# gist-ailab/QuBER

Hardware: AMD Instinct MI355X
Metric: refined masks/sec on 640x480 RGB-D (N=20 inst) (higher is better)
Workload: dtype f32; 1 GPU; batch=16 640x480 RGB-D, 20 initial instances/frame, ResNet-50 RGB-D refiner (boundary-error -> fg/centre/offset), encode+network+grouping+mask extraction; parallelism=dp1, hipgraph=False, foreground_filter=False

## Files before the change

quber_amd/csrc/api_ops.hip:

```cpp
#include "plan.h"

using namespace quber;

static float* g_op_ws = nullptr;
static int g_op_skip_rows = 0;
static int g_op_bf16 = 0;
static const size_t g_op_ws_floats = (size_t)256 << 20;
static int g_op_wino_reuse = 0;

bool quber::op_set_tuning(int key, int value) {
    if (key == 2) {
        if (value && !g_op_ws) {
            if (hipMalloc((void**)&g_op_ws, sizeof(float) * g_op_ws_floats) != hipSuccess) g_op_ws = nullptr;
        } else if (!value && g_op_ws) {
            (void)hipFree(g_op_ws);
            g_op_ws = nullptr;
        }
        return true;
    }
    if (key == 26) { g_op_wino_reuse = value; return true; }
    if (key == 12) { g_op_bf16 = value; return true; }
    if (key == 11) { g_op_skip_rows = value; return true; }
    return false;
}
// ... 86 lines not shown
    p.bf16 = 2; p.es = 2;
    return launch_conv(p, 1, (hipStream_t)stream);
}

int quber_op_conv2d_f16(const void* x, int32_t B, int32_t h, int32_t w, int32_t cin, const void* w_packed, int32_t cout, int32_t ksize, int32_t stride, int32_t pad, int32_t dil,
                        int32_t kmode, const float* scale, const float* shift, const void* residual, int32_t relu, double* gn_sums, int32_t gn_groups, void* y, void* stream) {
    if (cin % 8 || (kmode && cin % 64)) return fail("conv2d_f16: cin must be a multiple of 8 (slice-major K order: of 64)");
    if (ksize < 1 || stride < 1 || dil < 1 || pad < 0) return fail("conv2d_f16: bad geometry");
    ConvP p{};
    p.in = (const float*)x; p.w = (const float*)w_packed; p.scale = scale; p.shift = shift; p.res = (const float*)residual; p.out = (float*)y;
    conv_geometry(p, B, h, w, cin, cout, ksize, stride, pad, dil);
    if (p.OH < 1 || p.OW < 1) return fail("conv2d_f16: empty output");
    p.res_cs = cout; p.Kpad = (p.K + 63) / 64 * 64; p.relu = relu;
    p.kmode = kmode; p.bf16 = 2; p.es = 2;
    p.w_gs = (long)cout * p.Kpad; p.ss_gs = cout;
    if (gn_sums) {
        if (gn_groups < 1 || cout % gn_groups) return fail("conv2d_f16: channels must divide into the norm groups");
        p.gn_sum = gn_sums; p.gn_groups = gn_groups; p.gn_cpg = cout / gn_groups;
    }
    return launch_conv(p, 1, (hipStream_t)stream);
}

int quber_op_conv1x1_dual(const float* y, const float* x, int32_t B, int32_t oh, int32_t ow, int32_t mid, int32_t h2, int32_t w2, int32_t cin, int32_t stride,
                          const float* w, const float* shift, const float* ones, int32_t cout, int32_t relu, float* out, void* stream) {
    ConvP p{};
    p.in = y; p.in2 = x; p.w = w; p.scale = ones; p.shift = shift; p.out = out;
    conv_geometry(p, B, oh, ow, mid, cout, 1, 1, 0, 1);
    p.H2 = h2; p.W2 = w2; p.in2_cs = cin; p.stride2 = stride; p.K1 = mid;
    p.K = mid + cin; p.Kpad = mid + cin; p.relu = relu;
    p.bf16 = g_op_bf16; p.ss_gs = 0;
    p.ws = g_op_ws; p.ws_floats = g_op_ws ? g_op_ws_floats : 0;
    if (g_op_bf16 == 3 && tune().x8) {
        static PlaneScratch scratch;
        const int rs = scratch.split(w, (long)cout * p.Kpad, p, "conv1x1_dual", (hipStream_t)stream);
        if (rs) return rs;
    }
    const int rc = launch_conv_dual(p, 1, (hipStream_t)stream);
    if (rc == 1) return fail("conv1x1_dual: launch not covered by the dual kernel (workspace: tuning key 2)");
    return rc;
}

int quber_op_conv3x3_winograd(const float* x, int32_t B, int32_t h, int32_t w, int32_t cin, const float* w_oihw, int32_t cout, int32_t dil, int32_t m,
                              const float* scale, const float* shift, int32_t relu, float* u, float* ws, int64_t ws_floats, float* y, void* stream) {
    hipStream_t st = (hipStream_t)stream;
    if (!winograd_eligible(3, 1, dil, dil, cin, cout)) return fail("winograd: unsupported channel counts");
    if ((scale == nullptr) != (shift == nullptr)) return fail("winograd: scale and shift go together");
    if (m != 2 && m != 4 && m != 6) return fail("winograd: the output tile edge is 2, 4 or 6");
    int rc = g_op_wino_reuse ? 0 : launch_winograd_weights(w_oihw, cout, cin, m, u, st);
    if (rc) return rc;
    WinoP q{};
    q.in = mkview(x, B, h, w, cin); q.out = mkview(y, B, h, w, cout);
    q.u = u; q.scale = scale; q.shift = shift; q.ss_gs = 0; q.relu = relu; q.dil = dil; q.m = m;
    q.dtype = g_op_bf16;
    q.ws = ws; q.ws_floats = (size_t)ws_floats;
    if (m == 4 && tune().wino_fused && cout % 32 == 0 && (size_t)ws_floats >= (size_t)36 * cout * cin) {
        q.uf = ws;
        if (winograd_fused_ok(q, B, 1)) {
            rc = winograd_fused_prepare();
            if (rc) return rc;
            rc = g_op_wino_reuse ? 0 : launch_winograd_fused_pack(u, cout, cin, ws, st);
            if (rc) return rc;
            q.ws = ws + (size_t)36 * cout * cin; q.ws_floats = (size_t)ws_floats - (size_t)36 * cout * cin;
        } else {
            q.uf = nullptr;
        }
    }
    q.splitk_ws = g_op_ws; q.splitk_floats = g_op_ws ? g_op_ws_floats : 0;
    return launch_conv_winograd(q, B, 1, st);
}

int quber_op_groupnorm(const float* x, int32_t B, int32_t h, int32_t w, int32_t c, int32_t groups, const float* gamma,
                       const float* beta, float eps, int32_t relu, double* stats, float* y, void* stream) {
    View in = mkview(x, B, h, w, c), out = mkview(y, B, h, w, c);
    int rc = launch_gn_stats(in, B, 1, groups, stats, (hipStream_t)stream);
    if (rc) return rc;
    return launch_gn_apply(in, out, B, 1, groups, stats, gamma, beta, 0, eps, relu, (hipStream_t)stream);
}

int quber_op_bilinear(const float* x, int32_t B, int32_t h, int32_t w, int32_t c, int32_t oh, int32_t ow, float* y,
                      void* stream) {
    if (c % 4) return fail("bilinear: channels must be a multiple of 4");
    return launch_bilinear(mkview(x, B, h, w, c), mkview(y, B, oh, ow, c), B, (hipStream_t)stream);
}

int quber_op_group_pixels(const float* logits, int32_t n_planes, int32_t batch, int32_t h, int32_t w, int32_t cap,
                          const int32_t* centers, const int32_t* ncenters, uint8_t* ids, uint32_t* area, void* stream) {
    if (!logits || !centers || !ncenters || !ids || !area || batch < 1 || h < 1 || w < 1) return fail("bad argument to quber_op_group_pixels");
    return launch_group_pixels(logits, n_planes, batch, h, w, cap, centers, ncenters, ids, area, (hipStream_t)stream);
}

int quber_op_maxpool3x3s2(const float* x, int32_t B, int32_t h, int32_t w, int32_t c, float* y, void* stream) {
    if (c % 4) return fail("maxpool: channels must be a multiple of 4");
    return launch_maxpool3x3s2(mkview(x, B, h, w, c), mkview(y, B, (h + 1) / 2, (w + 1) / 2, c), B, 1, (hipStream_t)stream);
}

}
```

quber_amd/csrc/common.h:

```cpp
#pragma once
#include <hip/hip_runtime.h>
#include <stdint.h>
#include <string>

namespace quber {

struct View {
    float* p = nullptr;
    int B = 0, H = 0, W = 0, C = 0;
    int cs = 0;
    long gs = 0;
    int es = 4;
    float* at(long elems) const { return p ? reinterpret_cast<float*>(reinterpret_cast<char*>(p) + elems * es) : nullptr; }
};

struct ConvP {
    const float* in;
    const float* w;
    const float* scale;
    const float* shift;
    const float* res;
    const float* prelu;
    float* out;
    int B, H, W, Cin, in_cs;
// ... 21 lines not shown
    const char* tag;
    int pk_T, pk_tpg, pk_min, pk_in_bytes, pk_debug;
    const float* in2;
    int in2_cs, H2, W2, stride2, K1, pk_in2_bytes;
    long in2_gs;
    int es;
    int acc_chunk;
    int lean_in_bytes;
    unsigned dv_m[5], dv_s[5];
    const void* w3;
    long w3_plane;
    int dil_g[4];
    int h8_ss_bytes;
    const double* n_stats; const float* n_gamma; const float* n_beta; float* n_coef;
    int n_groups, n_param_gs, n_relu, n_coef_bytes; float n_eps;
    int bf16;
    int zones, zx1, zx2;
};

int device_cus();
void set_error(const std::string& msg);
int fail(const std::string& msg);

struct ProfScope {
    int rec;
    hipStream_t st;
    ProfScope(const char* tag, double bytes, double flops, hipStream_t s);
    ~ProfScope();
    ProfScope(const ProfScope&) = delete;
    ProfScope& operator=(const ProfScope&) = delete;
};

struct WinoNorm {
    const double* stats;
    const float* gamma;
    const float* beta;
    int groups, cpg, param_gs, relu;
    double n;
    float eps;
};

struct WinoP {
    View in, out;
    const float* u;
    const void* u3;
    long u3_plane;
    const float* uf;
    int algo;
    const float* scale;
    const float* shift;
    int ss_gs, relu;
    int dil;
    int m;
    int dtype;
    double* gn_sum;
    int gn_groups;
    WinoNorm norm;
    float* ws;
    size_t ws_floats;
    float* splitk_ws;
    size_t splitk_floats;
};

int launch_conv(const ConvP& p, int G, hipStream_t st);
int launch_conv_winograd(const WinoP& q, int B, int G, hipStream_t st);
int launch_winograd_weights(const float* w_oihw, int Cout, int Cin, int m, float* u, hipStream_t st);
void winograd_weights_host(const float* w_oihw, int Cout, int Cin, int m, float* u);
bool winograd_eligible(int k, int stride, int pad, int dil, int Cin, int Cout);
bool winograd_m6_channels_ok(int Cin, int Cout);
size_t winograd_ws_floats(int B, int H, int W, int Cin, int Cout, int G, int dil, int m);
double winograd_mac_ratio(int H, int W, int dil, int m);
bool winograd_fused_ok(const WinoP& q, int B, int G);
int launch_conv_winograd_fused(const WinoP& q, int B, int G, hipStream_t st);
void winograd_fused_pack_host(const float* u, int Cout, int Cin, float* uf);
int launch_winograd_fused_pack(const float* u, int Cout, int Cin, float* uf, hipStream_t st);
size_t winograd_fused_ws_floats(int B, int Cin, int G);
int winograd_fused_prepare();

struct Tuning {
    int winograd = 0;
    int wino_min_cin = 32;
    int wino_max_ratio = 67;
    int wino_variant = 0;
    int wino_min_cout = 32;
    int wino_pairs = 0;
    int wino_chunk_mb = 0;
    int wino_fused = 1;
    int wino_fused_max_cin = 160;
    int acc_chunk = 2;
    int tile_128x64 = 1;
    int force_tile = 0;
    int force_split = 0;
    int tail_split = 1;
    int persist = 1;
    int persist_min_nk = 32;
    int persist_min_tiles = 256;
    int persist_debug = 0;
    int stem_fused = 1;
    int lean_loader = 1;
    int fuse_shortcut = 1;
    int lanes = 1;
    int h8 = 1;
    int x8 = 1;
    int x8_min_nk = 8;
    int x8_min_rounds = 2;
    int zone_cols = 1;
    int small_n_64 = 1;
    int aspp_lanes = 1;
    int h8_narrow = 1;
    int h8_norm = 1;
    int h8_min_tiles = 224;
};
extern Tuning g_tune;
extern thread_local const Tuning* t_tune;
inline const Tuning& tune() { return t_tune ? *t_tune : g_tune; }
struct TuneScope {
    const Tuning* prev;
    explicit TuneScope(const Tuning* t) : prev(t_tune) { t_tune = t; }
    ~TuneScope() { t_tune = prev; }
    TuneScope(const TuneScope&) = delete;
    TuneScope& operator=(const TuneScope&) = delete;
};
bool tuning_set(Tuning& t, int key, int value);
template <int BM, int BN, int WM, int WN> int launch_conv_persistent(ConvP p, int G, int bpc, hipStream_t st);
size_t conv_persistent_ws_floats(int BM, int BN, int bpc);
bool conv_persistent_ok(const ConvP& p);
int conv_persistent_segments(int T, int P, int nk, int min_slices, int bid, int* out4, int cap);
int conv_persistent_fixup(int T, int P, int nk, int min_slices, int xcd, int j, int* tile, int* slots, int cap);
int launch_conv_dual(ConvP p, int G, hipStream_t st);
bool conv_h8_patch_takes(const ConvP& p, int G, bool norm);
int launch_conv_x8(ConvP p, int G, hipStream_t st);
int launch_split_bf16x3(const float* w, long n, void* planes, hipStream_t st);
int launch_conv_h8(ConvP p, int G, hipStream_t st);
#ifdef PK_STAMPS
int pk_read_stamps(unsigned long long* dst, int n);
int pk_read_span(unsigned long long* dst, int n);
#endif
int launch_preprocess(const uint8_t* rgb, const uint8_t* depth, const float* offs, const View& x, int B, int Bcap,
                      int H, int W, const float* mean6, const float* std6, int streams, hipStream_t st);
// ... 110 lines not shown
```

quber_amd/csrc/plan.hip:

```cpp
#include "plan.h"

namespace quber {
namespace {

constexpr int BLOCKS50[4] = {3, 4, 6, 3}, BLOCKS101[4] = {3, 4, 23, 3}, BLOCKS152[4] = {3, 8, 36, 3};

struct BnFold {
    const float *w, *b, *m, *v;
    bool ok() const { return w && b && m && v; }
    float scale(int o) const { return w[o] * (1.0f / sqrtf(v[o] + 1e-5f)); }
    float shift(int o, float sc) const { return b[o] - m[o] * sc; }
};
BnFold frozen_bn(Builder& b, const std::string& n, int C) {
    return {b.hw(n + ".norm.weight", C), b.hw(n + ".norm.bias", C), b.hw(n + ".norm.running_mean", C), b.hw(n + ".norm.running_var", C)};
}

struct WinoChoice { bool take = false; int m = 0; double ratio = 0.0; bool one_kernel = false; };
WinoChoice choose_winograd(int H, int W, int k, int stride, int pad, int dil, int Cin, int Cout, bool plain, int dtype) {
    WinoChoice r;
    if (!winograd_eligible(k, stride, pad, dil, Cin, Cout) || !plain || tune().winograd == 1 || (dtype != 0 && dtype != 3)) return r;
    const double lim = (double)tune().wino_max_ratio / 100.0;
    const double r6 = winograd_m6_channels_ok(Cin, Cout) ? winograd_mac_ratio(H, W, dil, 6) : 1e9;
    const double r4 = winograd_mac_ratio(H, W, dil, 4), r2 = winograd_mac_ratio(H, W, dil, 2);
    double best = lim;
// ... 83 lines not shown
    const int K = k * k * Cin, Kpad = (K + KS - 1) / KS * KS;
    const int OH = (in.H + 2 * pad - dil * (k - 1) - 1) / stride + 1;
    const int OW = (in.W + 2 * pad - dil * (k - 1) - 1) / stride + 1;
    const bool skip_rows = k == 3 && stride == 1 && dil > 1 && Cin % KS == 0 && cin_real == Cin && 10 * 2 * pad >= 2 * 3 * OH &&
                           !(winograd_eligible(k, stride, pad, dil, Cin, out.C) && !res && prelu.empty() &&
                             std::min(winograd_mac_ratio(in.H, in.W, dil, 4), winograd_mac_ratio(in.H, in.W, dil, 2)) <= tune().wino_max_ratio / 100.0 && tune().winograd != 1);
    const int kmode = (k > 1 && Cin % KS == 0 && !skip_rows) ? 1 : 0;
    if (dry) return;
    const double fl = 2.0 * OH * OW * (double)cin_real * k * k * Cout * G;
    c->flops += fl;
    if (OH != out.H || OW != out.W) { if (err.empty()) err = "internal: conv output geometry mismatch at " + name; return; }
    for (const float* p : w)
        if (!p) return;
    std::vector<float> packed((size_t)G * Cout * Kpad, 0.f);
    for (int g = 0; g < G; ++g)
        for (int o = 0; o < Cout; ++o) {
            float* dst = &packed[((size_t)g * Cout + o) * Kpad];
            for (int ci = 0; ci < cin_real; ++ci)
                for (int t = 0; t < k * k; ++t) {
                    const size_t kk = kmode ? ((size_t)(ci / KS) * k * k + t) * KS + ci % KS : (size_t)t * Cin + ci;
                    dst[kk] = w[g][((size_t)o * cin_real + ci) * k * k + t];
                }
        }
    ConvP p{};
    p.in = in.p;
    p.w = upload_weights(packed);
    if (aes != 2 && k == 1) { p.w3 = split3(p.w, packed.size()); p.w3_plane = (long)packed.size(); }
    p.es = aes;
    if (in.es != aes || out.es != aes || (res && res->es != aes)) { if (err.empty()) err = "internal: element type mismatch at " + name; return; }
    const bool ident = !affine && aes == 2 && Cout >= 32;
    p.scale = affine ? upload(scale) : ident ? upload(std::vector<float>((size_t)G * Cout, 1.f)) : nullptr;
    p.shift = affine ? upload(shift) : ident ? upload(std::vector<float>((size_t)G * Cout, 0.f)) : nullptr;
    for (size_t g = 0; g < dil_g.size() && g < 4; ++g) p.dil_g[g] = dil_g[g];
    p.prelu = prelu.empty() ? nullptr : upload(prelu);
    p.res = res ? res->p : nullptr;
    p.out = out.p;
    p.H = in.H; p.W = in.W; p.Cin = Cin; p.in_cs = in.cs;
    p.OH = OH; p.OW = OW; p.Cout = Cout; p.out_cs = out.cs;
    p.res_cs = res ? res->cs : 0;
    p.K = K; p.Kpad = Kpad;
    p.kh = k; p.kw = k; p.stride = stride; p.pad = pad; p.dil = dil;
    p.relu = relu; p.kmode = kmode; p.skip_rows = skip_rows;
    p.bf16 = c->cfg.compute_dtype;
    p.in_gs = in.gs; p.out_gs = out.gs; p.res_gs = res ? res->gs : 0;
    p.w_gs = (long)Cout * Kpad; p.ss_gs = Cout;
    p.ohw = OH * OW;
    quber_ctx* ctx = c;
    const WinoChoice wc = choose_winograd(in.H, in.W, k, stride, pad, dil, Cin, Cout, cin_real == Cin && !res && prelu.empty(), c->cfg.compute_dtype);
    const bool wino = wc.take;
    WinoP wq{};
    if (wino) {
        const int m = wc.m, P = (m + 2) * (m + 2);
        c->wino_flops += fl;
        c->wino_saved += fl * (1.0 - wc.ratio);
        c->wino_pad += fl * (wc.ratio - (double)((m + 2) * (m + 2)) / (9.0 * m * m));
        std::vector<float> u((size_t)G * P * Cout * Cin);
        for (int g = 0; g < G; ++g) winograd_weights_host(w[g], Cout, Cin, m, &u[(size_t)g * P * Cout * Cin]);
        wq.in = in; wq.out = out; wq.u = upload(u);
        wq.u3 = split3(wq.u, u.size()); wq.u3_plane = (long)u.size();
        if (wc.one_kernel) {
            std::vector<float> uf(u.size());
            for (int g = 0; g < G; ++g) winograd_fused_pack_host(&u[(size_t)g * P * Cout * Cin], Cout, Cin, &uf[(size_t)g * P * Cout * Cin]);
            wq.uf = upload(uf);
        }
        wq.scale = p.scale; wq.shift = p.shift; wq.ss_gs = Cout; wq.relu = relu; wq.dil = dil; wq.m = m;
        wq.dtype = c->cfg.compute_dtype;
    }
    std::shared_ptr<DeferredNorm> norm, norm16;
    if (wino && pending_norm && pending_norm->out.p == in.p && pending_norm->C == Cin && pending_norm->G == G) {
        norm = pending_norm;
        norm->absorbed = true;
    }
    float* coef16 = nullptr;
    if (!wino && aes == 2 && tune().h8_norm && tune().h8 && tune().h8_narrow && pending_norm && pending_norm->out.p == in.p && pending_norm->C == Cin &&
        pending_norm->G == G && k == 3 && stride == 1 && pad == 1 && dil == 1 && dil_g.empty() && Cin % 64 == 0 && Cin >= 128 && Cin <= 512 && cin_real == Cin &&
        (Cout == 128 || Cout == 64 || Cout == 32 || (Cout >= 256 && Cout % 8 == 0 && tune().h8_narrow != 2)) && !res && prelu.empty() && in.cs == pending_norm->in.cs && in.gs == pending_norm->in.gs) {
        norm16 = pending_norm;
        norm16->absorbed = true;
        coef16 = (float*)dalloc_bytes(sizeof(float) * (size_t)G * Bmax * Cin * 2);
    }
    pending_norm.reset();
    if (wino) {
        WinoP probe = wq;
        if (norm) probe.in = norm->in;
        const bool fusedk = wq.uf && winograd_fused_ok(probe, Bmax, G);
        wq.algo = fusedk ? 2 : 1;
        if (wq.uf && winograd_fused_prepare() && err.empty()) err = "winograd (fused): cannot raise the kernels' LDS limit";
        const size_t need = fusedk ? winograd_fused_ws_floats(Bmax, Cin, G) : winograd_ws_floats(Bmax, in.H, in.W, Cin, Cout, G, dil, wq.m);
        if (need > c->wino_floats) c->wino_floats = need;
        if (cur_lane) {
            const int lb = std::min(Bmax, LANE_BATCH);
            const size_t ln = fusedk ? winograd_fused_ws_floats(lb, Cin, G) : winograd_ws_floats(lb, in.H, in.W, Cin, Cout, G, dil, wq.m);
            if (ln > c->lane_wino_floats[cur_lane]) c->lane_wino_floats[cur_lane] = ln;
        }
    }
    auto fuse = std::make_shared<GnFuse>();
    last_conv = {fuse, out.p, G, Cout};
    const int L = cur_lane;
    c->ops.push_back({[p, G, ctx, fuse, wq, wino, norm, norm16, coef16, L](int B, hipStream_t st) mutable {
        const bool side = L && ctx->lane_now == L;
        float* const sk_ws = side ? ctx->lane_splitk_ws[L] : ctx->splitk_ws;
        const size_t sk_floats = side ? ctx->lane_splitk_floats : ctx->splitk_floats;
        if (wino) {
            wq.ws = side ? ctx->lane_wino_ws[L] : ctx->wino_ws; wq.ws_floats = side ? ctx->lane_wino_floats[L] : ctx->wino_floats;
            wq.splitk_ws = sk_ws; wq.splitk_floats = sk_floats;
            wq.gn_sum = fuse->sums; wq.gn_groups = fuse->groups;
            if (norm) {
                wq.in = norm->in;
                wq.norm = WinoNorm{norm->stats, norm->gamma, norm->beta, 32, 0, norm->C, 1, 0.0, 1e-5f};
            }
            return launch_conv_winograd(wq, B, G, st);
        }
        p.B = B;
        p.M = B * p.OH * p.OW;
        p.ws = sk_ws;
        p.ws_floats = sk_floats;
        p.gn_sum = fuse->sums;
        p.gn_groups = fuse->groups;
        p.gn_cpg = fuse->groups ? p.Cout / fuse->groups : 0;
        if (norm16) {
            ConvP q = p;
            q.in = norm16->in.p;
            q.n_stats = norm16->stats; q.n_gamma = norm16->gamma; q.n_beta = norm16->beta; q.n_coef = coef16;
            q.n_groups = 32; q.n_param_gs = norm16->C; q.n_relu = 1; q.n_eps = 1e-5f;
            if (conv_h8_patch_takes(q, G, true)) return launch_conv(q, G, st);
            const int rc = launch_gn_apply(norm16->in, norm16->out, B, G, 32, norm16->stats, norm16->gamma, norm16->beta, norm16->C, 1e-5f, 1, st);
            if (rc) return rc;
        }
        return launch_conv(p, G, st);
    }, OP_CONV, name, fl, 1});
    c->ops.back().lane = cur_lane;
}

void Builder::conv(const std::vector<std::string>& names, const View& in, int cin_real, const View& out, int k, int stride, int pad, int dil, Affine af, const View* res, bool relu,
                   const std::vector<int>& dil_g) {
    const int G = (int)names.size(), Cout = out.C;
    std::vector<float> scale((size_t)G * Cout, 1.f), shift((size_t)G * Cout, 0.f);
    std::vector<const float*> w;
    for (int g = 0; g < G; ++g) {
// ... 469 lines not shown
```

quber_amd/csrc/runtime.hip:

```cpp
#include <atomic>

#include "plan.h"

namespace quber {

Tuning g_tune;
thread_local const Tuning* t_tune = nullptr;

struct TuneKey { int key; int Tuning::*field; bool plan; };
constexpr TuneKey TUNE_KEYS[] = {
    {3, &Tuning::force_split, false},           {4, &Tuning::force_tile, false},
    {5, &Tuning::tail_split, false},            {6, &Tuning::winograd, true},
    {7, &Tuning::wino_min_cin, true},           {8, &Tuning::wino_max_ratio, true},
    {9, &Tuning::wino_variant, true},           {10, &Tuning::wino_min_cout, true},
    {13, &Tuning::persist, false},              {14, &Tuning::persist_min_nk, false},
    {15, &Tuning::persist_min_tiles, false},    {16, &Tuning::persist_debug, false},
    {17, &Tuning::wino_pairs, false},           {18, &Tuning::fuse_shortcut, true},
    {19, &Tuning::tile_128x64, false},          {20, &Tuning::wino_chunk_mb, false},
    {21, &Tuning::acc_chunk, false},            {24, &Tuning::lanes, false},
    {25, &Tuning::wino_fused, true},            {27, &Tuning::wino_fused_max_cin, true},
    {29, &Tuning::stem_fused, true},            {30, &Tuning::lean_loader, false},
    {31, &Tuning::h8, false},                   {32, &Tuning::h8_min_tiles, false},
    {35, &Tuning::x8, false},                   {36, &Tuning::x8_min_rounds, false},
    {37, &Tuning::x8_min_nk, false},            {38, &Tuning::h8_narrow, false},
    {39, &Tuning::h8_norm, true},               {41, &Tuning::aspp_lanes, true},
    {42, &Tuning::small_n_64, false},           {43, &Tuning::zone_cols, false},
};
int* tuning_field(Tuning& t, int key) {
    for (const TuneKey& k : TUNE_KEYS)
        if (k.key == key) return &(t.*k.field);
    return nullptr;
}
bool tuning_set(Tuning& t, int key, int value) {
    int* f = tuning_field(t, key);
    if (f) *f = value;
    return f != nullptr;
}
bool tuning_plan_time(int key) {
    for (const TuneKey& k : TUNE_KEYS)
        if (k.key == key) return k.plan;
    return false;
}

int device_cus() {
    static std::atomic<int> cache[64];
    int dev = 0;
    if (hipGetDevice(&dev) != hipSuccess) return -1;
    const bool cached = dev >= 0 && dev < 64;
    if (cached) {
        const int v = cache[dev].load(std::memory_order_relaxed);
        if (v > 0) return v;
    }
    hipDeviceProp_t prop;
    if (hipGetDeviceProperties(&prop, dev) != hipSuccess) return -1;
    const int cus = prop.multiProcessorCount > 0 ? prop.multiProcessorCount : 256;
    if (cached) cache[dev].store(cus, std::memory_order_relaxed);
    return cus;
}

static thread_local std::string g_err;
extern "C" const char* quber_last_error(void) { return g_err.c_str(); }
void set_error(const std::string& m) { g_err = m; }
int fail(const std::string& m) { g_err = m; return -1; }

thread_local Profiler* g_prof = nullptr;

ProfScope::ProfScope(const char* tag, double bytes, double flops, hipStream_t s) : rec(-1), st(s) {
    Profiler* p = g_prof;
    if (!p) return;
    int ti = -1;
    for (size_t i = 0; i < p->tags.size(); ++i)
        if (p->tags[i] == tag) { ti = (int)i; break; }
    if (ti < 0) { ti = (int)p->tags.size(); p->tags.emplace_back(tag); }
    ProfRec r{ti, p->get(), p->get(), bytes, flops};
    if (!r.e0 || !r.e1 || hipEventRecord(r.e0, s) != hipSuccess) return;
    rec = (int)p->recs.size();
    p->recs.push_back(r);
}
ProfScope::~ProfScope() {
// ... 5 lines not shown
```

quber_amd/csrc/winograd.hip:

```cpp
#include "common.h"
#include "winograd_xf.h"

namespace quber {

using namespace wxf;


namespace {

#ifndef QB_WINO_IN_WAVES44
#define QB_WINO_IN_WAVES44 2
#endif
constexpr int wino_in_waves(int O, int V) { return O == 4 ? (V == 4 ? QB_WINO_IN_WAVES44 : 5) : O == 2 ? 4 : 2; }
constexpr int wino_out_waves(int O, int V) { return O == 4 ? (V == 4 ? 2 : 3) : O == 2 ? 4 : 1; }

template <int O, int V, bool NORM>
__global__ __launch_bounds__(256) __attribute__((amdgpu_waves_per_eu(wino_in_waves(O, V)))) void wino_input_kernel(const float* __restrict__ in, int B, int H, int W, int CV, int in_cs,
                                                         long in_gs, int TH, int TW, int d, float* __restrict__ v, long v_gs,
                                                         const WinoNorm np, int Ball, int boff) {
    constexpr int T = O + 2;
    using VT = Vec<V>;
    const int g = blockIdx.z;
    in += g * in_gs;
    v += g * v_gs;
    const int tpb = 256 / CV;
    const int cv = tpb ? threadIdx.x % CV : blockIdx.y * 256 + threadIdx.x;
    const long tiles = (long)B * d * d * TH * TW;
    const int nblk = gridDim.x, xcd = blockIdx.x & 7, bq = nblk >> 3, br = nblk & 7;
    const int vb = (xcd < br ? xcd * (bq + 1) : br * (bq + 1) + (xcd - br) * bq) + (blockIdx.x >> 3);
    const long tile = tpb ? (long)vb * tpb + threadIdx.x / CV : vb;
    if (tile >= tiles || cv >= CV || (tpb && (int)(threadIdx.x / CV) >= tpb)) return;
    const TileAt ta = locate(tile, TH, TW, d);
    const int c = cv * V;
    const float* base = in + (long)ta.b * H * W * in_cs + c;
    VT nsc, nbi;
    if constexpr (NORM) {
        const double* sb = np.stats + (((long)g * Ball + boff + ta.b) * np.groups + c / np.cpg) * 2;
        const double mean = sb[0] / np.n;
        double var = sb[1] / np.n - mean * mean;
        if (var < 0.0) var = 0.0;
        const float rstd = (float)(1.0 / sqrt(var + (double)np.eps));
        const VT ga = vload<V>(np.gamma + g * np.param_gs + c), be = vload<V>(np.beta + g * np.param_gs + c);
#pragma unroll
        for (int e = 0; e < V; ++e) {
            nsc.v[e] = rstd * ga.v[e];
            nbi.v[e] = be.v[e] - (float)mean * nsc.v[e];
        }
    }
    const float relu_lo = (NORM && np.relu) ? 0.f : -__builtin_inff();
    VT t[T][T];
#pragma unroll
    for (int j = 0; j < T; ++j) {
        const int x = d * (O * ta.tx - 1 + j) + ta.px;
        VT col[T], tc[T];
        const int xc = min(max(x, 0), W - 1);
        const bool xin = (unsigned)x < (unsigned)W;
#pragma unroll
        for (int i = 0; i < T; ++i) {
            const int y = d * (O * ta.ty - 1 + i) + ta.py;
            col[i] = vload<V>(base + ((long)min(max(y, 0), H - 1) * W + xc) * in_cs);
        }
#pragma unroll
        for (int i = 0; i < T; ++i) {
            const int y = d * (O * ta.ty - 1 + i) + ta.py;
            const bool inside = xin && (unsigned)y < (unsigned)H;
#pragma unroll
            for (int e = 0; e < V; ++e) {
                float q = col[i].v[e];
                if constexpr (NORM) q = fmaxf(fmaf(q, nsc.v[e], nbi.v[e]), relu_lo);
                col[i].v[e] = inside ? q : 0.f;
            }
        }
        bt<O>(col, tc);
#pragma unroll
        for (int i = 0; i < T; ++i) t[i][j] = tc[i];
    }
    float* dst = v + tile * (long)(CV * V) + c;
    const long ps = tiles * (long)(CV * V);
#pragma unroll
    for (int i = 0; i < T; ++i) {
        VT row[T];
        bt<O>(t[i], row);
#pragma unroll
        for (int j = 0; j < T; ++j) vstore<V>(dst + (i * T + j) * ps, row[j]);
    }
}

constexpr int OUT_ITERS = 4;
template <int O, int V>
__global__ __launch_bounds__(256) __attribute__((amdgpu_waves_per_eu(wino_out_waves(O, V)))) void wino_output_kernel(const float* __restrict__ m, long m_gs, int B, int OH, int OW, int CV,
                                                          int TH, int TW, int d, const float* __restrict__ scale,
                                                          const float* __restrict__ shift, int ss_gs, int relu,
                                                          float* __restrict__ out, int out_cs, long out_gs,
                                                          double* __restrict__ gn_sum, int gn_groups, int gn_cpg, int Ball, int boff, int iters) {
    constexpr int T = O + 2;
    using VT = Vec<V>;
    const int g = blockIdx.z;
    m += g * m_gs;
    out += g * out_gs;
    const int tpb = 256 / CV;
    const int cv = tpb ? threadIdx.x % CV : blockIdx.y * 256 + threadIdx.x;
    const int c = cv * V;
    const long per_img = (long)d * d * TH * TW;
    const long tiles = (long)B * per_img;
    const int step = tpb ? tpb : 1;
    const long tile0 = (long)blockIdx.x * step * iters;
    const bool lane_ok = cv < CV && (!tpb || (int)(threadIdx.x / CV) < tpb);
    __shared__ double gacc[2 * 32 * 2];
    const int b0 = (int)(tile0 / per_img);
    if (gn_sum) {
        if (threadIdx.x < 128) gacc[threadIdx.x] = 0.0;
        __syncthreads();
    }
    double s0 = 0.0, q0 = 0.0, s1 = 0.0, q1 = 0.0;
    const long ps = tiles * (long)(CV * V);
    VT sc, sh;
    if (scale && lane_ok) {
        sc = vload<V>(scale + g * ss_gs + c);
        sh = vload<V>(shift + g * ss_gs + c);
    }
    for (int it = 0; it < iters; ++it) {
        const long tile = tile0 + (long)it * step + (tpb ? threadIdx.x / CV : 0);
        if (!lane_ok || tile >= tiles) continue;
        const TileAt ta = locate(tile, TH, TW, d);
        const float* src = m + tile * (long)(CV * V) + c;
        VT s[O][T];
#pragma unroll
        for (int j = 0; j < T; ++j) {
            VT col[T], sj[O];
#pragma unroll
            for (int i = 0; i < T; ++i) col[i] = vload<V>(src + (i * T + j) * ps);
            at<O>(col, sj);
#pragma unroll
            for (int i = 0; i < O; ++i) s[i][j] = sj[i];
        }
        double a = 0.0, q = 0.0;
#pragma unroll
        for (int i = 0; i < O; ++i) {
            const int oy = d * (O * ta.ty + i) + ta.py;
            VT row[O];
            at<O>(s[i], row);
            if (oy >= OH) continue;
#pragma unroll
            for (int j = 0; j < O; ++j) {
                const int ox = d * (O * ta.tx + j) + ta.px;
                if (ox >= OW) continue;
                VT y = row[j];
#pragma unroll
                for (int e = 0; e < V; ++e) {
                    if (scale) y.v[e] = fmaf(y.v[e], sc.v[e], sh.v[e]);
                    if (relu) y.v[e] = fmaxf(y.v[e], 0.f);
                    a += (double)y.v[e];
                    q += (double)y.v[e] * y.v[e];
                }
                vstore<V>(out + (((long)ta.b * OH + oy) * OW + ox) * out_cs + c, y);
            }
        }
        if (ta.b == b0) { s0 += a; q0 += q; } else { s1 += a; q1 += q; }
    }
    if (gn_sum) {
        if (lane_ok) {
            const int grp = c / gn_cpg;
            if (s0 != 0.0 || q0 != 0.0) { atomicAdd(&gacc[grp * 2], s0); atomicAdd(&gacc[grp * 2 + 1], q0); }
            if (s1 != 0.0 || q1 != 0.0) { atomicAdd(&gacc[64 + grp * 2], s1); atomicAdd(&gacc[64 + grp * 2 + 1], q1); }
        }
        __syncthreads();
        if (threadIdx.x < 128) {
            const double v = gacc[threadIdx.x];
            const int b = b0 + (threadIdx.x >> 6);
            if (v != 0.0 && b < B) atomicAdd(&gn_sum[(((long)g * Ball + boff + b) * gn_groups) * 2 + (threadIdx.x & 63)], v);
        }
    }
}

template <int O>
__host__ __device__ inline void gmul(double a, double b, double c, double* y) {
    if constexpr (O == 2) {
        y[0] = a;
        y[1] = 0.5 * (a + b + c);
        y[2] = 0.5 * (a - b + c);
        y[3] = c;
    } else if constexpr (O == 4) {
        y[0] = a * (64.0 / 81.0);
        y[1] = -a * (128.0 / 243.0) - b * (32.0 / 81.0) - c * (8.0 / 27.0);
        y[2] = -a * (128.0 / 243.0) + b * (32.0 / 81.0) - c * (8.0 / 27.0);
        y[3] = a * (32.0 / 243.0) + b * (16.0 / 81.0) + c * (8.0 / 27.0);
        y[4] = a * (32.0 / 243.0) - b * (16.0 / 81.0) + c * (8.0 / 27.0);
        y[5] = c;
    } else {
        y[0] = a;
        y[1] = -(a + b + c) * (2.0 / 9.0);
        y[2] = -(a - b + c) * (2.0 / 9.0);
        y[3] = a / 90.0 + b / 45.0 + c * (2.0 / 45.0);
        y[4] = a / 90.0 - b / 45.0 + c * (2.0 / 45.0);
        y[5] = (32.0 * a + 16.0 * b + 8.0 * c) / 45.0;
        y[6] = (32.0 * a - 16.0 * b + 8.0 * c) / 45.0;
        y[7] = c;
    }
}
// ... 15 lines not shown
    constexpr int P = (O + 2) * (O + 2);
    const long n = (long)Cout * Cin;
    for (long i = blockIdx.x * (long)blockDim.x + threadIdx.x; i < n; i += (long)gridDim.x * blockDim.x) {
        double up[P];
        wino_filter<O>(w + i * 9, up);
        for (int p = 0; p < P; ++p) u[p * n + i] = (float)up[p];
    }
}

template <int O>
void weights_host(const float* w_oihw, int Cout, int Cin, float* u) {
    constexpr int P = (O + 2) * (O + 2);
    for (int o = 0; o < Cout; ++o)
        for (int c = 0; c < Cin; ++c) {
            double up[P];
            wino_filter<O>(w_oihw + ((size_t)o * Cin + c) * 9, up);
            for (int p = 0; p < P; ++p) u[((size_t)p * Cout + o) * Cin + c] = (float)up[p];
        }
}

}

void winograd_weights_host(const float* w_oihw, int Cout, int Cin, int m, float* u) {
    if (m == 6) weights_host<6>(w_oihw, Cout, Cin, u);
    else if (m == 4) weights_host<4>(w_oihw, Cout, Cin, u);
    else weights_host<2>(w_oihw, Cout, Cin, u);
}

int launch_winograd_weights(const float* w_oihw, int Cout, int Cin, int m, float* u, hipStream_t st) {
    if (m == 6) hipLaunchKernelGGL(wino_weight_kernel<6>, dim3(256), dim3(256), 0, st, w_oihw, Cout, Cin, u);
    else if (m == 4) hipLaunchKernelGGL(wino_weight_kernel<4>, dim3(256), dim3(256), 0, st, w_oihw, Cout, Cin, u);
    else hipLaunchKernelGGL(wino_weight_kernel<2>, dim3(256), dim3(256), 0, st, w_oihw, Cout, Cin, u);
    QB_CHECK(hipGetLastError());
    return 0;
}

bool winograd_m6_channels_ok(int Cin, int Cout) {
    return (Cin / 2 <= 256 || (Cin / 2) % 256 == 0) && (Cout / 2 <= 256 || (Cout / 2) % 256 == 0);
}

bool winograd_eligible(int k, int stride, int pad, int dil, int Cin, int Cout) {
    return k == 3 && stride == 1 && dil >= 1 && pad == dil && Cin % 32 == 0 && Cout % 4 == 0 && Cin >= tune().wino_min_cin &&
           Cout >= tune().wino_min_cout && (Cin / 4 <= 256 || (Cin / 4) % 256 == 0) && (Cout / 4 <= 256 || (Cout / 4) % 256 == 0);
}

size_t winograd_ws_floats(int B, int H, int W, int Cin, int Cout, int G, int dil, int m) {
    const size_t tiles = (size_t)B * wino_tiles(H, W, dil, m);
    return (size_t)G * (m + 2) * (m + 2) * tiles * (size_t)(Cin + Cout);
}

double winograd_mac_ratio(int H, int W, int dil, int m) {
    return (double)((m + 2) * (m + 2)) * wino_tiles(H, W, dil, m) / (9.0 * H * W);
}


template <int O, int V>
static int run_winograd(const WinoP& q, int Ball, int G, hipStream_t st) {
    constexpr int P = (O + 2) * (O + 2);
    const View& in = q.in;
    const View& out = q.out;
    const int H = in.H, W = in.W, Cin = in.C, Cout = out.C, d = q.dil;
    const int TH = tiles_1d(H, d, O), TW = tiles_1d(W, d, O);
    const long tiles_pf = wino_tiles(H, W, d, O);
    if ((long)Ball * tiles_pf * P >= (1L << 31) / 2) return fail("winograd: too many tiles");
    int cb = Ball;
    if (tune().wino_chunk_mb > 0) {
        const double per_frame = 4.0 * G * P * (double)tiles_pf * (Cin + Cout);
        cb = (int)((double)tune().wino_chunk_mb * 1048576.0 / per_frame);
        if (cb < 1) cb = 1;
        if (cb > Ball) cb = Ball;
        cb = (Ball + (Ball + cb - 1) / cb - 1) / ((Ball + cb - 1) / cb);
    }
    if (winograd_ws_floats(cb, H, W, Cin, Cout, G, d, O) > q.ws_floats) return fail("winograd: workspace too small");
    WinoNorm np = q.norm;
    if (np.stats) {
        if (np.groups <= 0 || Cin % np.groups || (Cin / np.groups) % 4) return fail("winograd: fused GroupNorm needs 4 | channels per group");
        np.cpg = Cin / np.groups;
        np.n = (double)H * W * np.cpg;
    }
    const int CVo = Cout / V, per_iter = CVo <= 256 ? 256 / CVo : 1;
    int iters = OUT_ITERS;
    {
        const long groups = CVo <= 256 ? ((long)Ball * tiles_pf + per_iter - 1) / per_iter : (long)Ball * tiles_pf * (CVo / 256);
        while (iters > 1 && groups * G / iters < 2048) iters >>= 1;
    }
    const bool gn_here = q.gn_sum && q.gn_groups > 0 && q.gn_groups <= 32 && (Cout / q.gn_groups) % 4 == 0 &&
                         tiles_pf >= (long)per_iter * iters;
    for (int b0 = 0; b0 < Ball; b0 += cb) {
        const int B = Ball - b0 < cb ? Ball - b0 : cb;
        const long tiles = (long)B * tiles_pf;
        float* v = q.ws;
        auto grid = [&](int CV) {
            return CV <= 256 ? dim3((unsigned)((tiles + 256 / CV - 1) / (256 / CV)), 1, G) : dim3((unsigned)tiles, CV / 256, G);
        };
        const float* in_p = in.p + (size_t)b0 * H * W * in.cs;
        float* out_p = out.p + (size_t)b0 * H * W * out.cs;
        const bool shared_v = G > 1 && in.gs == 0 && !np.stats;
        const int Gv = shared_v ? 1 : G;
        float* m = q.ws + (size_t)Gv * P * tiles * Cin;
        auto grid_v = [&](int CV) {
            return CV <= 256 ? dim3((unsigned)((tiles + 256 / CV - 1) / (256 / CV)), 1, Gv) : dim3((unsigned)tiles, CV / 256, Gv);
        };
        {
            ProfScope prof("wino_input", 4.0 * Gv * Cin * ((double)B * H * W + (double)P * tiles), 0.0, st);
            if (np.stats)
                hipLaunchKernelGGL((wino_input_kernel<O, V, true>), grid_v(Cin / V), dim3(256), 0, st, in_p, B, H, W, Cin / V, in.cs, in.gs, TH,
                                   TW, d, v, (long)P * tiles * Cin, np, Ball, b0);
            else
                hipLaunchKernelGGL((wino_input_kernel<O, V, false>), grid_v(Cin / V), dim3(256), 0, st, in_p, B, H, W, Cin / V, in.cs, in.gs, TH,
                                   TW, d, v, (long)P * tiles * Cin, np, Ball, b0);
        }
        QB_CHECK(hipGetLastError());
        ConvP p{};
        p.in = v; p.w = q.u; p.out = m;
        p.w3 = q.u3; p.w3_plane = q.u3_plane;
        p.B = 1; p.H = (int)tiles; p.W = 1; p.Cin = Cin; p.in_cs = Cin;
        p.OH = (int)tiles; p.OW = 1; p.Cout = Cout; p.out_cs = Cout;
        p.K = Cin; p.Kpad = Cin;
        p.kh = 1; p.kw = 1; p.stride = 1; p.pad = 0; p.dil = 1;
        p.M = (int)tiles; p.ohw = (int)tiles;
        p.in_gs = tiles * Cin; p.out_gs = tiles * Cout; p.w_gs = (long)Cout * Cin;
        p.ws = q.splitk_ws; p.ws_floats = q.splitk_floats;
        p.tag = "wino_gemm";
        p.bf16 = q.dtype == 3 ? 3 : 0;
        if (shared_v) {
            for (int g = 0; g < G; ++g) {
                p.w = q.u + (size_t)g * P * Cout * Cin;
                if (q.u3) p.w3 = reinterpret_cast<const unsigned short*>(q.u3) + (size_t)g * P * Cout * Cin;
                p.out = m + (size_t)g * P * tiles * Cout;
                const int rc = launch_conv(p, P, st);
                if (rc) return rc;
            }
        } else {
            const int rc = launch_conv(p, G * P, st);
            if (rc) return rc;
        }
        dim3 og = grid(CVo);
        og.x = (og.x + iters - 1) / iters;
        {
            ProfScope prof("wino_output", 4.0 * G * Cout * ((double)P * tiles + (double)B * H * W), 0.0, st);
            hipLaunchKernelGGL((wino_output_kernel<O, V>), og, dim3(256), 0, st, m, (long)P * tiles * Cout, B, H, W, CVo, TH, TW, d,
                               q.scale, q.shift, q.ss_gs, q.relu, out_p, out.cs, out.gs, gn_here ? q.gn_sum : nullptr, q.gn_groups,
                               q.gn_groups ? Cout / q.gn_groups : 1, Ball, b0, iters);
        }
        QB_CHECK(hipGetLastError());
    }
    if (q.gn_sum && !gn_here) return launch_gn_stats(out, Ball, G, q.gn_groups, q.gn_sum, st, false);
    return 0;
}

int launch_conv_winograd(const WinoP& q, int B, int G, hipStream_t st) {
    const View& in = q.in;
    const View& out = q.out;
    if (!winograd_eligible(3, 1, q.dil, q.dil, in.C, out.C) || out.H != in.H || out.W != in.W || (q.m != 2 && q.m != 4 && q.m != 6))
        return fail("winograd: unsupported geometry");
    if (q.m == 6 && !winograd_m6_channels_ok(in.C, out.C)) return fail("winograd: channel counts unsupported by the 6x6 variant");
    if (in.cs % 4 || out.cs % 4 || ((uintptr_t)in.p & 15) || ((uintptr_t)out.p & 15) || (in.gs & 3) || (out.gs & 3))
        return fail("winograd: operands must be 16-byte aligned");
    if (q.algo == 2 || (q.algo == 0 && winograd_fused_ok(q, B, G))) return launch_conv_winograd_fused(q, B, G, st);
    if (q.m == 4 && tune().wino_pairs && winograd_m6_channels_ok(in.C, out.C)) return run_winograd<4, 2>(q, B, G, st);
    return q.m == 6 ? run_winograd<6, 2>(q, B, G, st) : q.m == 4 ? run_winograd<4, 4>(q, B, G, st) : run_winograd<2, 4>(q, B, G, st);
}

}
```

quber_amd/csrc/winograd_xf.h:

```cpp
#pragma once
#include "common.h"

namespace quber {
namespace wxf {

template <int V>
struct Vec {
    float v[V];
    __device__ inline Vec operator+(const Vec& o) const { Vec r; for (int e = 0; e < V; ++e) r.v[e] = v[e] + o.v[e]; return r; }
    __device__ inline Vec operator-(const Vec& o) const { Vec r; for (int e = 0; e < V; ++e) r.v[e] = v[e] - o.v[e]; return r; }
};
template <int V>
__device__ inline Vec<V> operator*(float s, const Vec<V>& a) { Vec<V> r; for (int e = 0; e < V; ++e) r.v[e] = s * a.v[e]; return r; }
template <int V>
__device__ inline Vec<V> vzero() { Vec<V> r; for (int e = 0; e < V; ++e) r.v[e] = 0.f; return r; }
template <int V>
__device__ inline Vec<V> vload(const float* p) {
    Vec<V> r;
    if constexpr (V == 4) { const float4 t = *reinterpret_cast<const float4*>(p); r.v[0] = t.x; r.v[1] = t.y; r.v[2] = t.z; r.v[3] = t.w; }
    else { const float2 t = *reinterpret_cast<const float2*>(p); r.v[0] = t.x; r.v[1] = t.y; }
    return r;
}
template <int V>
__device__ inline void vstore(float* p, const Vec<V>& a) {
// ... 36 lines not shown
__device__ inline void at(const T* x, T* y) {
    if constexpr (O == 2) {
        y[0] = (x[0] + x[1]) + x[2];
        y[1] = (x[1] - x[2]) - x[3];
    } else if constexpr (O == 4) {
        const T a = x[1] + x[2], b = x[1] - x[2], c = x[3] + x[4], d = x[3] - x[4];
        y[0] = (x[0] + a) + c;
        y[1] = 0.75f * b + 1.5f * d;
        y[2] = 0.5625f * a + 2.25f * c;
        y[3] = (0.421875f * b + 3.375f * d) + x[5];
    } else {
        const T s1 = x[1] + x[2], d1 = x[1] - x[2], s2 = x[3] + x[4], d2 = x[3] - x[4], s3 = x[5] + x[6], d3 = x[5] - x[6];
        y[0] = ((x[0] + s1) + s2) + s3;
        y[1] = (d1 + 2.f * d2) + 0.5f * d3;
        y[2] = (s1 + 4.f * s2) + 0.25f * s3;
        y[3] = (d1 + 8.f * d2) + 0.125f * d3;
        y[4] = (s1 + 16.f * s2) + 0.0625f * s3;
        y[5] = ((d1 + 32.f * d2) + 0.03125f * d3) + x[7];
    }
}

struct TileAt { int b, py, px, ty, tx; };
__device__ inline TileAt locate(long tile, int TH, int TW, int d) {
    TileAt t;
    t.tx = tile % TW;
    long r = tile / TW;
    t.ty = r % TH;
    r /= TH;
    t.px = r % d;
    r /= d;
    t.py = r % d;
    t.b = (int)(r / d);
    return t;
}


__device__ inline TileAt locate32(unsigned tile, unsigned TH, unsigned TW, unsigned d) {
    TileAt t;
    unsigned r = tile / TW;
    t.tx = (int)(tile - r * TW);
    unsigned r2 = r / TH;
    t.ty = (int)(r - r2 * TH);
    unsigned r3 = r2 / d;
    t.px = (int)(r2 - r3 * d);
    const unsigned r4 = r3 / d;
    t.py = (int)(r3 - r4 * d);
    t.b = (int)r4;
    return t;
}

inline int tiles_1d(int n, int d, int m) { return ((n + d - 1) / d + m - 1) / m; }
inline long wino_tiles(int H, int W, int d, int m) { return (long)d * d * tiles_1d(H, d, m) * tiles_1d(W, d, m); }

}
}
```

Measured before the change: 10020 refined masks/s.

## Pack dilated Winograd phases contiguously along each axis to cut padded tiles

Adds a packed tiling mode for dilated Winograd convolutions. The dilation phases are laid end-to-end along each axis with shared single-pixel separators, instead of each phase getting its own rounded-up tile grid. This reduces the number of tiles, and so the padding waste in the input transform, batched GEMM and output transform. The input and output kernels gain a template path that walks the packed axis positions. It is on by default through a new tuning key, and per-tile index arithmetic becomes more complex.

```diff
diff --git a/quber_amd/csrc/api_ops.hip b/quber_amd/csrc/api_ops.hip
--- a/quber_amd/csrc/api_ops.hip
+++ b/quber_amd/csrc/api_ops.hip
@@ -162,6 +162,7 @@
     q.in = mkview(x, B, h, w, cin); q.out = mkview(y, B, h, w, cout);
     q.u = u; q.scale = scale; q.shift = shift; q.ss_gs = 0; q.relu = relu; q.dil = dil; q.m = m;
     q.dtype = g_op_bf16;
+    q.pack = tune().wino_pack;
     q.ws = ws; q.ws_floats = (size_t)ws_floats;
     if (m == 4 && tune().wino_fused && cout % 32 == 0 && (size_t)ws_floats >= (size_t)36 * cout * cin) {
         q.uf = ws;
diff --git a/quber_amd/csrc/common.h b/quber_amd/csrc/common.h
--- a/quber_amd/csrc/common.h
+++ b/quber_amd/csrc/common.h
@@ -97,6 +97,7 @@
     int ss_gs, relu;
     int dil;
     int m;
+    int pack;
     int dtype;
     double* gn_sum;
     int gn_groups;
@@ -115,6 +116,7 @@
 bool winograd_m6_channels_ok(int Cin, int Cout);
 size_t winograd_ws_floats(int B, int H, int W, int Cin, int Cout, int G, int dil, int m);
 double winograd_mac_ratio(int H, int W, int dil, int m);
+double winograd_mac_ratio_run(int H, int W, int dil, int m, bool pack);
 bool winograd_fused_ok(const WinoP& q, int B, int G);
 int launch_conv_winograd_fused(const WinoP& q, int B, int G, hipStream_t st);
 void winograd_fused_pack_host(const float* u, int Cout, int Cin, float* uf);
@@ -130,6 +132,7 @@
     int wino_min_cout = 32;
     int wino_pairs = 0;
     int wino_chunk_mb = 0;
+    int wino_pack = 1;
     int wino_fused = 1;
     int wino_fused_max_cin = 160;
     int acc_chunk = 2;
diff --git a/quber_amd/csrc/plan.hip b/quber_amd/csrc/plan.hip
--- a/quber_amd/csrc/plan.hip
+++ b/quber_amd/csrc/plan.hip
@@ -159,8 +159,6 @@
     if (wino) {
         const int m = wc.m, P = (m + 2) * (m + 2);
         c->wino_flops += fl;
-        c->wino_saved += fl * (1.0 - wc.ratio);
-        c->wino_pad += fl * (wc.ratio - (double)((m + 2) * (m + 2)) / (9.0 * m * m));
         std::vector<float> u((size_t)G * P * Cout * Cin);
         for (int g = 0; g < G; ++g) winograd_weights_host(w[g], Cout, Cin, m, &u[(size_t)g * P * Cout * Cin]);
         wq.in = in; wq.out = out; wq.u = upload(u);
@@ -172,6 +170,7 @@
         }
         wq.scale = p.scale; wq.shift = p.shift; wq.ss_gs = Cout; wq.relu = relu; wq.dil = dil; wq.m = m;
         wq.dtype = c->cfg.compute_dtype;
+        wq.pack = tune().wino_pack;
     }
     std::shared_ptr<DeferredNorm> norm, norm16;
     if (wino && pending_norm && pending_norm->out.p == in.p && pending_norm->C == Cin && pending_norm->G == G) {
@@ -192,6 +191,9 @@
         if (norm) probe.in = norm->in;
         const bool fusedk = wq.uf && winograd_fused_ok(probe, Bmax, G);
         wq.algo = fusedk ? 2 : 1;
+        const double ratio = fusedk ? wc.ratio : winograd_mac_ratio_run(in.H, in.W, dil, wq.m, wq.pack != 0);
+        c->wino_saved += fl * (1.0 - ratio);
+        c->wino_pad += fl * (ratio - (double)((wq.m + 2) * (wq.m + 2)) / (9.0 * wq.m * wq.m));
         if (wq.uf && winograd_fused_prepare() && err.empty()) err = "winograd (fused): cannot raise the kernels' LDS limit";
         const size_t need = fusedk ? winograd_fused_ws_floats(Bmax, Cin, G) : winograd_ws_floats(Bmax, in.H, in.W, Cin, Cout, G, dil, wq.m);
         if (need > c->wino_floats) c->wino_floats = need;
diff --git a/quber_amd/csrc/runtime.hip b/quber_amd/csrc/runtime.hip
--- a/quber_amd/csrc/runtime.hip
+++ b/quber_amd/csrc/runtime.hip
@@ -25,6 +25,7 @@
     {37, &Tuning::x8_min_nk, false},            {38, &Tuning::h8_narrow, false},
     {39, &Tuning::h8_norm, true},               {41, &Tuning::aspp_lanes, true},
     {42, &Tuning::small_n_64, false},           {43, &Tuning::zone_cols, false},
+    {51, &Tuning::wino_pack, true},
 };
 int* tuning_field(Tuning& t, int key) {
     for (const TuneKey& k : TUNE_KEYS)
diff --git a/quber_amd/csrc/winograd.hip b/quber_amd/csrc/winograd.hip
--- a/quber_amd/csrc/winograd.hip
+++ b/quber_amd/csrc/winograd.hip
@@ -14,10 +14,10 @@
 constexpr int wino_in_waves(int O, int V) { return O == 4 ? (V == 4 ? QB_WINO_IN_WAVES44 : 5) : O == 2 ? 4 : 2; }
 constexpr int wino_out_waves(int O, int V) { return O == 4 ? (V == 4 ? 2 : 3) : O == 2 ? 4 : 1; }
 
-template <int O, int V, bool NORM>
+template <int O, int V, bool NORM, bool PK>
 __global__ __launch_bounds__(256) __attribute__((amdgpu_waves_per_eu(wino_in_waves(O, V)))) void wino_input_kernel(const float* __restrict__ in, int B, int H, int W, int CV, int in_cs,
                                                          long in_gs, int TH, int TW, int d, float* __restrict__ v, long v_gs,
-                                                         const WinoNorm np, int Ball, int boff) {
+                                                         const WinoNorm np, int Ball, int boff, const Axis ay, const Axis ax) {
     constexpr int T = O + 2;
     using VT = Vec<V>;
     const int g = blockIdx.z;
@@ -25,12 +25,28 @@
     v += g * v_gs;
     const int tpb = 256 / CV;
     const int cv = tpb ? threadIdx.x % CV : blockIdx.y * 256 + threadIdx.x;
-    const long tiles = (long)B * d * d * TH * TW;
+    const long tiles = PK ? (long)B * TH * TW : (long)B * d * d * TH * TW;
     const int nblk = gridDim.x, xcd = blockIdx.x & 7, bq = nblk >> 3, br = nblk & 7;
     const int vb = (xcd < br ? xcd * (bq + 1) : br * (bq + 1) + (xcd - br) * bq) + (blockIdx.x >> 3);
     const long tile = tpb ? (long)vb * tpb + threadIdx.x / CV : vb;
     if (tile >= tiles || cv >= CV || (tpb && (int)(threadIdx.x / CV) >= tpb)) return;
-    const TileAt ta = locate(tile, TH, TW, d);
+    TileAt ta;
+    int yy[T];
+    AxisPos sx{0, 0};
+    if constexpr (PK) {
+        const long per_img = (long)TH * TW;
+        ta.b = (int)(tile / per_img);
+        const int local = (int)(tile - ta.b * per_img), aty = local / TW;
+        AxisPos sy = axis_begin(ay, aty);
+#pragma unroll
+        for (int i = 0; i < T; ++i) {
+            yy[i] = axis_coord(ay, sy);
+            sy = axis_next(ay, sy);
+        }
+        sx = axis_begin(ax, local - aty * TW);
+    } else {
+        ta = locate(tile, TH, TW, d);
+    }
     const int c = cv * V;
     const float* base = in + (long)ta.b * H * W * in_cs + c;
     VT nsc, nbi;
@@ -51,18 +67,26 @@
     VT t[T][T];
 #pragma unroll
     for (int j = 0; j < T; ++j) {
-        const int x = d * (O * ta.tx - 1 + j) + ta.px;
+        int x;
+        if constexpr (PK) {
+            x = axis_coord(ax, sx);
+            sx = axis_next(ax, sx);
+        } else {
+            x = d * (O * ta.tx - 1 + j) + ta.px;
+        }
         VT col[T], tc[T];
         const int xc = min(max(x, 0), W - 1);
         const bool xin = (unsigned)x < (unsigned)W;
 #pragma unroll
         for (int i = 0; i < T; ++i) {
-            const int y = d * (O * ta.ty - 1 + i) + ta.py;
+            int y;
+            if constexpr (PK) y = yy[i]; else y = d * (O * ta.ty - 1 + i) + ta.py;
             col[i] = vload<V>(base + ((long)min(max(y, 0), H - 1) * W + xc) * in_cs);
         }
 #pragma unroll
         for (int i = 0; i < T; ++i) {
-            const int y = d * (O * ta.ty - 1 + i) + ta.py;
+            int y;
+            if constexpr (PK) y = yy[i]; else y = d * (O * ta.ty - 1 + i) + ta.py;
             const bool inside = xin && (unsigned)y < (unsigned)H;
 #pragma unroll
             for (int e = 0; e < V; ++e) {
@@ -87,12 +111,13 @@
 }
 
 constexpr int OUT_ITERS = 4;
-template <int O, int V>
+template <int O, int V, bool PK>
 __global__ __launch_bounds__(256) __attribute__((amdgpu_waves_per_eu(wino_out_waves(O, V)))) void wino_output_kernel(const float* __restrict__ m, long m_gs, int B, int OH, int OW, int CV,
                                                           int TH, int TW, int d, const float* __restrict__ scale,
                                                           const float* __restrict__ shift, int ss_gs, int relu,
                                                           float* __restrict__ out, int out_cs, long out_gs,
-                                                          double* __restrict__ gn_sum, int gn_groups, int gn_cpg, int Ball, int boff, int iters) {
+                                                          double* __restrict__ gn_sum, int gn_groups, int gn_cpg, int Ball, int boff, int iters,
+                                                          const Axis ay, const Axis ax) {
     constexpr int T = O + 2;
     using VT = Vec<V>;
     const int g = blockIdx.z;
@@ -101,7 +126,7 @@
     const int tpb = 256 / CV;
     const int cv = tpb ? threadIdx.x % CV : blockIdx.y * 256 + threadIdx.x;
     const int c = cv * V;
-    const long per_img = (long)d * d * TH * TW;
+    const long per_img = PK ? (long)TH * TW : (long)d * d * TH * TW;
     const long tiles = (long)B * per_img;
     const int step = tpb ? tpb : 1;
     const long tile0 = (long)blockIdx.x * step * iters;
@@ -122,7 +147,22 @@
     for (int it = 0; it < iters; ++it) {
         const long tile = tile0 + (long)it * step + (tpb ? threadIdx.x / CV : 0);
         if (!lane_ok || tile >= tiles) continue;
-        const TileAt ta = locate(tile, TH, TW, d);
+        TileAt ta;
+        int oys[O], oxs[O];
+        if constexpr (PK) {
+            ta.b = (int)(tile / per_img);
+            const int local = (int)(tile - ta.b * per_img), aty = local / TW;
+            AxisPos sy = axis_next(ay, axis_begin(ay, aty)), sx = axis_next(ax, axis_begin(ax, local - aty * TW));
+#pragma unroll
+            for (int i = 0; i < O; ++i) {
+                oys[i] = axis_coord(ay, sy);
+                oxs[i] = axis_coord(ax, sx);
+                sy = axis_next(ay, sy);
+                sx = axis_next(ax, sx);
+            }
+        } else {
+            ta = locate(tile, TH, TW, d);
+        }
         const float* src = m + tile * (long)(CV * V) + c;
         VT s[O][T];
 #pragma unroll
@@ -137,14 +177,16 @@
         double a = 0.0, q = 0.0;
 #pragma unroll
         for (int i = 0; i < O; ++i) {
-            const int oy = d * (O * ta.ty + i) + ta.py;
+            int oy;
+            if constexpr (PK) oy = oys[i]; else oy = d * (O * ta.ty + i) + ta.py;
             VT row[O];
             at<O>(s[i], row);
-            if (oy >= OH) continue;
+            if (oy >= OH || (PK && oy < 0)) continue;
 #pragma unroll
             for (int j = 0; j < O; ++j) {
-                const int ox = d * (O * ta.tx + j) + ta.px;
-                if (ox >= OW) continue;
+                int ox;
+                if constexpr (PK) ox = oxs[j]; else ox = d * (O * ta.tx + j) + ta.px;
+                if (ox >= OW || (PK && ox < 0)) continue;
                 VT y = row[j];
 #pragma unroll
                 for (int e = 0; e < V; ++e) {
@@ -266,6 +308,9 @@
 double winograd_mac_ratio(int H, int W, int dil, int m) {
     return (double)((m + 2) * (m + 2)) * wino_tiles(H, W, dil, m) / (9.0 * H * W);
 }
+double winograd_mac_ratio_run(int H, int W, int dil, int m, bool pack) {
+    return (double)((m + 2) * (m + 2)) * wino_tiles_run(H, W, dil, m, pack) / (9.0 * H * W);
+}
 
 
 template <int O, int V>
@@ -274,8 +319,10 @@
     const View& in = q.in;
     const View& out = q.out;
     const int H = in.H, W = in.W, Cin = in.C, Cout = out.C, d = q.dil;
-    const int TH = tiles_1d(H, d, O), TW = tiles_1d(W, d, O);
-    const long tiles_pf = wino_tiles(H, W, d, O);
+    const Axis ay = make_axis(H, d, O, q.pack != 0), ax = make_axis(W, d, O, q.pack != 0);
+    const bool pk = ay.packed || ax.packed;
+    const int TH = pk ? ay.T : tiles_1d(H, d, O), TW = pk ? ax.T : tiles_1d(W, d, O);
+    const long tiles_pf = (long)ay.T * ax.T;
     if ((long)Ball * tiles_pf * P >= (1L << 31) / 2) return fail("winograd: too many tiles");
     int cb = Ball;
     if (tune().wino_chunk_mb > 0) {
@@ -317,12 +364,12 @@
         };
         {
             ProfScope prof("wino_input", 4.0 * Gv * Cin * ((double)B * H * W + (double)P * tiles), 0.0, st);
-            if (np.stats)
-                hipLaunchKernelGGL((wino_input_kernel<O, V, true>), grid_v(Cin / V), dim3(256), 0, st, in_p, B, H, W, Cin / V, in.cs, in.gs, TH,
-                                   TW, d, v, (long)P * tiles * Cin, np, Ball, b0);
-            else
-                hipLaunchKernelGGL((wino_input_kernel<O, V, false>), grid_v(Cin / V), dim3(256), 0, st, in_p, B, H, W, Cin / V, in.cs, in.gs, TH,
-                                   TW, d, v, (long)P * tiles * Cin, np, Ball, b0);
+            auto launch_in = [&](auto kern) {
+                hipLaunchKernelGGL(kern, grid_v(Cin / V), dim3(256), 0, st, in_p, B, H, W, Cin / V, in.cs, in.gs, TH, TW, d, v, (long)P * tiles * Cin, np,
+                                   Ball, b0, ay, ax);
+            };
+            if (np.stats) pk ? launch_in(wino_input_kernel<O, V, true, true>) : launch_in(wino_input_kernel<O, V, true, false>);
+            else pk ? launch_in(wino_input_kernel<O, V, false, true>) : launch_in(wino_input_kernel<O, V, false, false>);
         }
         QB_CHECK(hipGetLastError());
         ConvP p{};
@@ -353,9 +400,11 @@
         og.x = (og.x + iters - 1) / iters;
         {
             ProfScope prof("wino_output", 4.0 * G * Cout * ((double)P * tiles + (double)B * H * W), 0.0, st);
-            hipLaunchKernelGGL((wino_output_kernel<O, V>), og, dim3(256), 0, st, m, (long)P * tiles * Cout, B, H, W, CVo, TH, TW, d,
-                               q.scale, q.shift, q.ss_gs, q.relu, out_p, out.cs, out.gs, gn_here ? q.gn_sum : nullptr, q.gn_groups,
-                               q.gn_groups ? Cout / q.gn_groups : 1, Ball, b0, iters);
+            auto launch_out = [&](auto kern) {
+                hipLaunchKernelGGL(kern, og, dim3(256), 0, st, m, (long)P * tiles * Cout, B, H, W, CVo, TH, TW, d, q.scale, q.shift, q.ss_gs, q.relu, out_p,
+                                   out.cs, out.gs, gn_here ? q.gn_sum : nullptr, q.gn_groups, q.gn_groups ? Cout / q.gn_groups : 1, Ball, b0, iters, ay, ax);
+            };
+            pk ? launch_out(wino_output_kernel<O, V, true>) : launch_out(wino_output_kernel<O, V, false>);
         }
         QB_CHECK(hipGetLastError());
     }
diff --git a/quber_amd/csrc/winograd_xf.h b/quber_amd/csrc/winograd_xf.h
--- a/quber_amd/csrc/winograd_xf.h
+++ b/quber_amd/csrc/winograd_xf.h
@@ -112,5 +112,52 @@
 inline int tiles_1d(int n, int d, int m) { return ((n + d - 1) / d + m - 1) / m; }
 inline long wino_tiles(int H, int W, int d, int m) { return (long)d * d * tiles_1d(H, d, m) * tiles_1d(W, d, m); }
 
+struct Axis {
+    int n, d, m;
+    int packed;
+    int T;
+    int Tp;
+    int q, rem;
+};
+__host__ __device__ inline int axis_tiles_phase(int n, int d, int m) { return d * (((n + d - 1) / d + m - 1) / m); }
+__host__ __device__ inline int axis_tiles_packed(int n, int d, int m) { return (n + (d < n ? d : n) - 1 + m - 1) / m; }
+__host__ __device__ inline Axis make_axis(int n, int d, int m, bool pack) {
+    Axis a;
+    a.n = n; a.d = d; a.m = m;
+    a.Tp = ((n + d - 1) / d + m - 1) / m;
+    const int tph = d * a.Tp, tpk = axis_tiles_packed(n, d, m);
+    a.packed = pack && tpk < tph;
+    a.T = a.packed ? tpk : tph;
+    a.q = n / d; a.rem = n % d;
+    return a;
+}
+struct AxisPos { int p, r; };
+__host__ __device__ inline AxisPos axis_begin(const Axis& a, int t) {
+    AxisPos s;
+    if (!a.packed) {
+        s.p = t / a.Tp;
+        s.r = a.m * (t - s.p * a.Tp) - 1;
+        return s;
+    }
+    const int e = a.m * t, head = a.rem * (a.q + 2);
+    const bool lng = e < head;
+    const int seg = lng ? a.q + 2 : a.q + 1, e2 = lng ? e : e - head, k = e2 / seg;
+    s.p = (lng ? 0 : a.rem) + k;
+    s.r = e2 - k * seg - 1;
+    return s;
+}
+__host__ __device__ inline AxisPos axis_next(const Axis& a, AxisPos s) {
+    ++s.r;
+    if (a.packed && s.r == a.q + (s.p < a.rem ? 1 : 0)) { ++s.p; s.r = -1; }
+    return s;
+}
+__host__ __device__ inline int axis_coord(const Axis& a, AxisPos s) {
+    const int c = a.d * s.r + s.p;
+    return (s.r >= 0 && s.p < a.d && c < a.n) ? c : -1;
+}
+inline long wino_tiles_run(int H, int W, int d, int m, bool pack) {
+    return (long)make_axis(H, d, m, pack).T * make_axis(W, d, m, pack).T;
+}
+
 }
 }
```

New measurement: 10200 refined masks/s (median of 6 runs). 1.9% higher.
